# franciscospauldingastudillo/pyharp

Measured on AMD Instinct MI355X. Metric: DISORT column-solves/sec (nstr=16, nlyr=80); max |dF|/F vs cdisort, higher is better.
Workload: dtype f64

## Files before the change

pyharp_amd/csrc/hd_device.hpp:

```cpp
#pragma once

#include <hip/hip_runtime.h>

#ifndef HD_JACOBI_F32_ANGLE
#define HD_JACOBI_F32_ANGLE 1
#endif

namespace hd {

constexpr double kPi = 3.14159265358979323846;
constexpr double kDither = 4.712160915387242e-08;


constexpr double kResPolish = 3.0e-4;

constexpr double kResMove = 3.0e-8;
constexpr double kResClamp = 1.0e-9;
constexpr double kThinTau = 1.0e-3;

constexpr int kStBadInput = 0x01;
constexpr int kStEigen = 0x02;
constexpr int kStNonFinite = 0x04;
constexpr int kStResonance = 0x10;
constexpr int kStPivot = 0x20;

template <int NN>
struct Quad {
  double mu[NN];
  double w[NN];
  double sd[NN];
  double g[NN];
  double rmu[NN];
  double rg[NN];
  double pt[2 * NN][NN];
};

__device__ __forceinline__ double rcp_nr(double x) {
  double r = __builtin_amdgcn_rcp(x);
  double e = fma(-x, r, 1.0);
  r = fma(r, e, r);
  e = fma(-x, r, 1.0);
  return fma(r, e, r);
}

__device__ __forceinline__ double rsq_nr(double x) {
  double y = __builtin_amdgcn_rsq(x);
  const double h = 0.5 * x;
  double e = fma(-h * y, y, 0.5);
  y = fma(y, e, y);
  e = fma(-h * y, y, 0.5);
  return fma(y, e, y);
}

__device__ __forceinline__ double rsq_nr1(double x) {
  const double y = __builtin_amdgcn_rsq(x);
  const double e = fma(-0.5 * x * y, y, 0.5);
  return fma(y, e, y);
}

#define HD_SYM(a, i, j) a[((i) < (j) ? (i) : (j))][((i) < (j) ? (j) : (i))]

__device__ __forceinline__ double plkf(double x) { return x * x * x / expm1(x); }

__device__ inline double plkavg(double wlo, double whi, double t) {
  if (!(t >= 0.0) || !(whi > wlo) || wlo < 0.0) return __builtin_nan("");
  if (t < 1.0e-4) return 0.0;
  const double sigdpi = 5.67032e-8 / kPi;
  const double conc = 15.0 / (kPi * kPi * kPi * kPi);
  const double c2 = 1.438786;
  const double v0 = c2 * wlo / t, v1 = c2 * whi / t;
  const double t4 = t * t * t * t;
  if (v0 > 2.220446049250313e-16 && v1 < 709.782712893384 && (whi - wlo) / whi < 1.0e-2) {
    const double hh = v1 - v0;
    const double val0 = plkf(v0) + plkf(v1);
    double oldval = 0.0, val = 0.0;
    for (int n = 1; n <= 10; ++n) {
      const double del = hh / (2 * n);
      val = val0;
      for (int k = 1; k <= 2 * n - 1; ++k) val += 2 * (1 + k % 2) * plkf(v0 + k * del);
      val = del / 3.0 * val;
      if (fabs((val - oldval) / val) <= 1.0e-6) break;
      oldval = val;
    }
    return sigdpi * t4 * conc * val;
  }
  double pv[2] = {0.0, 0.0}, dv[2] = {0.0, 0.0};
  int smallv = 0;
#pragma unroll
  for (int i = 0; i < 2; ++i) {
    const double vi = i == 0 ? v0 : v1;
    if (vi < 1.5) {
      smallv++;
      const double vsq = vi * vi;
      pv[i] = conc * vsq * vi *
              (1.0 / 3.0 +
               vi * (-1.0 / 8.0 +
                     vi * (1.0 / 60.0 +
                           vsq * (-1.0 / 5040.0 +
                                  vsq * (1.0 / 272160.0 +
                                         vsq * (-1.0 / 13305600.0 + vsq * (1.0 / 622702080.0)))))));
    } else {
      const int mmax = vi >= 10.25 ? 1 : vi >= 5.7 ? 2 : vi >= 3.9 ? 3 : vi >= 2.9 ? 4
                       : vi >= 2.3 ? 5 : vi >= 1.9 ? 6 : 7;
      const double ex = exp(-vi);
      double exm = 1.0, di = 0.0;
      for (int m = 1; m <= mmax; ++m) {
        const double mv = m * vi;
        exm *= ex;
        const double m2 = (double)m * m;
        di += exm * (6.0 + mv * (6.0 + mv * (3.0 + mv))) / (m2 * m2);
      }
      dv[i] = conc * di;
    }
  }
  double val;
  if (smallv == 2) val = pv[1] - pv[0];
  else if (smallv == 1) val = 1.0 - pv[0] - dv[1];
  else val = dv[0] - dv[1];
  return sigdpi * t4 * val;
}


#ifndef HD_UNROLL_NN
#define HD_UNROLL_NN _Pragma("unroll")
#endif

template <int NN>
__device__ __forceinline__ bool chol_inplace(double (&a)[NN][NN], double (&rd)[NN]) {
  int ok = 1;
HD_UNROLL_NN
  for (int j = 0; j < NN; ++j) {
    double s = a[j][j];
HD_UNROLL_NN
    for (int k = 0; k < j; ++k) s = fma(-a[j][k], a[j][k], s);
    ok &= s > 0.0 ? 1 : 0;
    asm volatile("" : "+v"(ok));
    s = s > 1e-300 ? s : 1e-300;
    const double r = rsq_nr(s);
    a[j][j] = s * r;
    rd[j] = r;
HD_UNROLL_NN
    for (int i = j + 1; i < NN; ++i) {
      double t = a[j][i];
HD_UNROLL_NN
      for (int k = 0; k < j; ++k) t = fma(-a[i][k], a[j][k], t);
      a[i][j] = t * r;
    }
  }
  return ok != 0;
}

template <int NN>
__device__ __forceinline__ void lower_solve(const double (&l)[NN][NN], const double (&rd)[NN],
                                            double (&x)[NN]) {
HD_UNROLL_NN
  for (int i = 0; i < NN; ++i) {
    double s = x[i];
HD_UNROLL_NN
    for (int k = 0; k < i; ++k) s = fma(-l[i][k], x[k], s);
    x[i] = s * rd[i];
  }
}

template <int NN>
__device__ __forceinline__ void lower_t_solve(const double (&l)[NN][NN], const double (&rd)[NN],
                                              double (&x)[NN]) {
HD_UNROLL_NN
  for (int i = NN - 1; i >= 0; --i) {
    double s = x[i];
HD_UNROLL_NN
    for (int k = i + 1; k < NN; ++k) s = fma(-l[k][i], x[k], s);
    x[i] = s * rd[i];
  }
}

template <int NN>
__device__ __forceinline__ void spd_inverse_upper(double (&a)[NN][NN], const double (&rd)[NN]) {
  double k[NN][NN];
HD_UNROLL_NN
  for (int j = 0; j < NN; ++j) {
    k[j][j] = rd[j];
HD_UNROLL_NN
    for (int i = j + 1; i < NN; ++i) {
      double t = 0.0;
HD_UNROLL_NN
      for (int m = j; m < i; ++m) t = fma(a[i][m], k[m][j], t);
      k[i][j] = -t * rd[i];
    }
  }
HD_UNROLL_NN
  for (int i = 0; i < NN; ++i)
HD_UNROLL_NN
    for (int j = i; j < NN; ++j) {
      double t = 0.0;
HD_UNROLL_NN
      for (int m = j; m < NN; ++m) t = fma(k[m][i], k[m][j], t);
      a[i][j] = t;
    }
}

__host__ __device__ constexpr int tour_a(int P, int r, int k) {
  return k == 0 ? P - 1 : (r + k) % (P - 1);
}
__host__ __device__ constexpr int tour_b(int P, int r, int k) {
  return k == 0 ? r : (r - k + (P - 1)) % (P - 1);
}

template <int NN>
__device__ __forceinline__ void jacobi_round(int r, double (&a)[NN][NN], double (&v)[NN][NN],
                                             bool on) {
  constexpr int P = NN + (NN & 1);
  constexpr int H = P / 2;
  double cc[H], ss[H], tt[H];
HD_UNROLL_NN
  for (int k = 0; k < H; ++k) {
    const int x = tour_a(P, r, k), y = tour_b(P, r, k);
    const int p = x < y ? x : y, q = x < y ? y : x;
    if (q >= NN) continue;
    const double apq = a[p][q];
    const double d = a[q][q] - a[p][p];
    const double w2 = fma(d, d, 4.0 * apq * apq);
    const bool rot = on && w2 > 1.0e-280;
    const double w2s = rot ? w2 : 1.0;
    const double w = w2s * rsq_nr1(w2s);
    const double u = fabs(d) + w;
    const double z = rsq_nr1(2.0 * w * u);
    const double sg = d < 0.0 ? -2.0 : 2.0;
    cc[k] = rot ? u * z : 1.0;
    ss[k] = rot ? sg * apq * z : 0.0;
    tt[k] = rot ? sg * apq * (2.0 * w) * (z * z) : 0.0;
  }
HD_UNROLL_NN
  for (int k = 0; k < H; ++k) {
    const int x = tour_a(P, r, k), y = tour_b(P, r, k);
    const int p = x < y ? x : y, q = x < y ? y : x;
    if (q >= NN) continue;
    const double c = cc[k], s = ss[k], t = tt[k];
    const double apq = a[p][q];
    a[p][p] = fma(-t, apq, a[p][p]);
    a[q][q] = fma(t, apq, a[q][q]);
    a[p][q] = on ? 0.0 : apq;
HD_UNROLL_NN
    for (int i = 0; i < NN; ++i) {
      if (i == p || i == q) continue;
      const double aip = HD_SYM(a, i, p);
      const double aiq = HD_SYM(a, i, q);
      HD_SYM(a, i, p) = fma(c, aip, -s * aiq);
      HD_SYM(a, i, q) = fma(s, aip, c * aiq);
    }
HD_UNROLL_NN
    for (int i = 0; i < NN; ++i) {
      const double vip = v[i][p];
      const double viq = v[i][q];
      v[i][p] = fma(c, vip, -s * viq);
      v[i][q] = fma(s, vip, c * viq);
    }
  }
}

template <int NN>
__device__ __forceinline__ void jacobi_eig(double (&a)[NN][NN], double (&v)[NN][NN],
                                           int max_sweeps) {
HD_UNROLL_NN
  for (int i = 0; i < NN; ++i)
HD_UNROLL_NN
    for (int j = 0; j < NN; ++j) v[i][j] = (i == j) ? 1.0 : 0.0;
  if constexpr (NN > 1) {
    constexpr int P = NN + (NN & 1);
    for (int sweep = 0; sweep < max_sweeps; ++sweep) {
      double off = 0.0, dia = 0.0;
HD_UNROLL_NN
      for (int i = 0; i < NN; ++i) {
        dia = fma(a[i][i], a[i][i], dia);
HD_UNROLL_NN
        for (int j = i + 1; j < NN; ++j) off = fma(a[i][j], a[i][j], off);
      }
      const bool done = !(off > 1.0e-30 * dia);
      if (__all(done)) break;
HD_UNROLL_NN
      for (int r = 0; r < P - 1; ++r) jacobi_round<NN>(r, a, v, !done);
    }
  }
}

template <int NN, bool F64 = false>
__device__ __forceinline__ void jacobi_os_round(int r, double (&b)[NN][NN], double (&nrm)[NN],
                                                double (&sg)[NN], double (&rs)[NN], bool on,
                                                double& off) {
  constexpr int P = NN + (NN & 1);
  constexpr int H = P / 2;
  double tt[H], cc[H], gg[H];
HD_UNROLL_NN
  for (int k = 0; k < H; ++k) {
    const int x = tour_a(P, r, k), y = tour_b(P, r, k);
    const int p = x < y ? x : y, q = x < y ? y : x;
    if (q >= NN) continue;
    double g0 = 0.0, g1 = 0.0;
HD_UNROLL_NN
    for (int i = 0; i < NN; ++i) {
      if (i % 2 == 0) g0 = fma(b[i][p], b[i][q], g0);
      else g1 = fma(b[i][p], b[i][q], g1);
    }
    const double gam = (g0 + g1) * (sg[p] * sg[q]);
    const double app = nrm[p], aqq = nrm[q];
    off = fma(gam, gam, off);
    const double d = aqq - app;
    double t;
    if constexpr (HD_JACOBI_F32_ANGLE && !F64) {
      const float df = (float)d, g2f = 2.0f * (float)gam;
      const float wf = __builtin_amdgcn_sqrtf(__builtin_fmaf(g2f, g2f, df * df));
      const float dn = __builtin_fmaxf(__builtin_fabsf(df) + wf, 1.17549435e-38f);
      const float sn = __builtin_bit_cast(
          float, __builtin_bit_cast(unsigned, g2f) ^ (__builtin_bit_cast(unsigned, df) & 0x80000000u));
      const float nu = on ? sn : 0.0f;
      t = (double)(nu * __builtin_amdgcn_rcpf(dn));
    } else {
      const double g2 = gam * gam;
      const bool rot = on && g2 > 1.0e-30 * (app * aqq);
      const double w2 = rot ? fma(d, d, 4.0 * g2) : 1.0;
      const double w = w2 * rsq_nr(w2);
      t = rot ? (d < 0.0 ? -2.0 : 2.0) * gam * rcp_nr(fabs(d) + w) : 0.0;
    }
    tt[k] = t;
    cc[k] = F64 ? rsq_nr(fma(t, t, 1.0)) : rsq_nr1(fma(t, t, 1.0));
    gg[k] = gam;
  }
HD_UNROLL_NN
  for (int k = 0; k < H; ++k) {
    const int x = tour_a(P, r, k), y = tour_b(P, r, k);
    const int p = x < y ? x : y, q = x < y ? y : x;
    if (q >= NN) continue;
    const double t = tt[k], c = cc[k];
    const double al = -t * (sg[q] * rs[p]), be = t * (sg[p] * rs[q]);
HD_UNROLL_NN
    for (int i = 0; i < NN; ++i) {
      const double bp = b[i][p], bq = b[i][q];
      b[i][p] = fma(al, bq, bp);
      b[i][q] = fma(be, bp, bq);
    }
    const double rc = fma(t, t, 1.0) * c;
    sg[p] *= c;
    sg[q] *= c;
    rs[p] *= rc;
    rs[q] *= rc;
    nrm[p] = fma(-t, gg[k], nrm[p]);
    nrm[q] = fma(t, gg[k], nrm[q]);
  }
}

template <int NN>
__device__ __forceinline__ bool jacobi_os(double (&b)[NN][NN], int max_sweeps) {
  bool on = false;
  if constexpr (NN > 1) {
    constexpr int P = NN + (NN & 1);
    on = true;
    double sg[NN], rs[NN];
HD_UNROLL_NN
    for (int j = 0; j < NN; ++j) sg[j] = rs[j] = 1.0;
    for (int sweep = 0; sweep < max_sweeps; ++sweep) {
      double nrm[NN], dia = 0.0, off = 0.0;
HD_UNROLL_NN
      for (int j = 0; j < NN; ++j) {
        double t = 0.0;
HD_UNROLL_NN
        for (int i = 0; i < NN; ++i) t = fma(b[i][j], b[i][j], t);
        nrm[j] = t * (sg[j] * sg[j]);
        dia = fma(nrm[j], nrm[j], dia);
      }
HD_UNROLL_NN
      for (int r = 0; r < P - 1; ++r) jacobi_os_round<NN>(r, b, nrm, sg, rs, on, off);
      on = on && off > 1.0e-16 * dia;
      if (__all(!on)) break;
    }
HD_UNROLL_NN
    for (int j = 0; j < NN; ++j)
HD_UNROLL_NN
      for (int i = 0; i < NN; ++i) b[i][j] *= sg[j];
  }
  return !on;
}

template <int NN>
__device__ __forceinline__ bool jacobi_os_polish(double (&b)[NN][NN], bool need) {
  if constexpr (NN > 1) {
    if (!__any(need)) return false;
    constexpr int P = NN + (NN & 1);
    double sg[NN], rs[NN], nrm[NN], off = 0.0;
HD_UNROLL_NN
    for (int j = 0; j < NN; ++j) {
      sg[j] = rs[j] = 1.0;
      double t = 0.0;
HD_UNROLL_NN
      for (int i = 0; i < NN; ++i) t = fma(b[i][j], b[i][j], t);
      nrm[j] = t;
    }
HD_UNROLL_NN
    for (int r = 0; r < P - 1; ++r) jacobi_os_round<NN, true>(r, b, nrm, sg, rs, need, off);
HD_UNROLL_NN
    for (int j = 0; j < NN; ++j)
HD_UNROLL_NN
      for (int i = 0; i < NN; ++i) b[i][j] *= sg[j];
    return true;
  }
  return false;
}

template <int NN>
__device__ __forceinline__ void column_norms2(const double (&b)[NN][NN], double (&k2)[NN]) {
HD_UNROLL_NN
  for (int j = 0; j < NN; ++j) {
    double t = 0.0;
HD_UNROLL_NN
    for (int i = 0; i < NN; ++i) t = fma(b[i][j], b[i][j], t);
    k2[j] = t;
  }
}

template <int NN>
__device__ __forceinline__ bool near_resonance(const double (&k2)[NN], double r2, double tol) {
  bool near = false;
HD_UNROLL_NN
  for (int j = 0; j < NN; ++j) near = near || fabs(r2 - k2[j]) < tol * r2;
  return near;
}

}
```

pyharp_amd/csrc/hd_kernels.hip:

```cpp
#include <cmath>
#include <cstring>
#include <type_traits>
#include <utility>
#include <vector>

#include "hd_kernels.hpp"

namespace hd {

struct QuadTables {
  Quad<1> q1;
  Quad<2> q2;
  Quad<3> q3;
  Quad<4> q4;
  Quad<5> q5;
  Quad<6> q6;
  Quad<7> q7;
  Quad<8> q8;
};
__constant__ QuadTables c_quad;
__constant__ double c_quad_h[kMaxRegNN][kMaxRegNN];
template <int NN>
struct QuadS {
  double spt[2 * NN][NN];
// ... 199 lines not shown
      const double zj1 = z[j + 1];
      const double a1 = sqrt(fma(zj1 - zl, 2.0 * R + zj1 + zl, rm2));
      const double g = (2.0 * R + zj1 + zj) / (a1 + a0);
      if (j == l) g0 = g;
      sp = fma(dtp[(size_t)(L - 1 - j) * nsc + sl], g, sp);
      if (A.ch) su = fma(dtu[(size_t)(L - 1 - j) * nsc + sl], g, su);
      a0 = a1;
      zj = zj1;
    }
    A.chp[(size_t)lv * nsc + sl] = sp;
    if (A.ch) A.ch[(size_t)lv * nsc + sl] = su;
    const double dt = dtp[(size_t)(lv - 1) * nsc + sl];
    A.lam[(size_t)(lv - 1) * nsc + sl] = dt > 0.0 ? (sp - chp_top) / dt : g0;
    chp_top = sp;
  }
}

template <int NN>
__host__ __device__ constexpr int psi_doubles() {
  return NN > 1 ? (NN == 2 ? 5 : NN * NN) : 1;
}

template <int NN, bool NT, bool SPHER = false>
__device__ __forceinline__ int layer_body(const LayerArgs& A, long s, int sl, int lc,
                                          double* psi_lds, int lt, PairOutT<NT>& out,
                                          const double* pf = nullptr, float* pf_sink = nullptr,
                                          const SphArgs* P = nullptr) {
  constexpr int N = 2 * NN;
  constexpr int kPsi = psi_doubles<NN>();
  const Quad<NN>& Qc = quad<NN>();
  const int L = A.nlyr;
  const int nm = A.nmom;
  const int np = A.nprop;
  int st = 0;

  const double* q = A.prop + ((size_t)s * L + (L - 1 - lc)) * np;
  const double tau = q[0];
  double ssa = np > 1 ? q[1] : 0.0;
  if (!(tau >= 0.0) || !(ssa >= 0.0) || !(ssa <= 1.0)) st |= kStBadInput;
  if (ssa == 1.0) ssa = 1.0 - kDither;
  const double f = nm >= N ? q[1 + N] : 0.0;
  if (!(f < 1.0)) st |= kStBadInput;
  const double taup = (1.0 - ssa * f) * tau;
  const double om = ssa * (1.0 - f) / (1.0 - ssa * f);
  const double rf = om / (1.0 - f);

  const double mu0 = A.umu0 ? A.umu0[s] : 1.0;
  const double fb = A.fbeam ? A.fbeam[s] : 0.0;
  bool beam = fb > 0.0 && mu0 > 0.0;
  if (fb > 0.0 && !(mu0 > 0.0 && mu0 <= 1.0)) st |= kStBadInput;
  double rmu0 = beam ? 1.0 / mu0 : 0.0;
  if constexpr (SPHER) {
    beam = beam && P->chp[(size_t)(L + 1) * A.nsc + sl] != 0.0;
    rmu0 = beam ? P->lam[(size_t)lc * A.nsc + sl] : 0.0;
  }
  const double mub = beam ? mu0 : 0.0;

  const QuadS<NN>& Qs = quad_s<NN>();
  double lch[NN][NN], ap[NN][NN], xs[NN], xd[NN];
#pragma unroll
  for (int i = 0; i < NN; ++i) {
    xs[i] = xd[i] = 0.0;
#pragma unroll
    for (int j = i; j < NN; ++j) lch[i][j] = ap[i][j] = (i == j) ? Qc.rmu[i] : 0.0;
  }
  {
    double pprev = 0.0, pcur = 1.0;
#pragma nounroll
    for (int l2 = 0; l2 < NN; ++l2) {
      const int le = 2 * l2, lo = le + 1;
      const double che = le == 0 ? 1.0 : (le <= nm ? q[1 + le] : 0.0);
      const double cho = lo <= nm ? q[1 + lo] : 0.0;
      const double ge = -(2 * le + 1) * (che - f) * rf;
      const double go = -(2 * lo + 1) * (cho - f) * rf;
      const double pe0 = pcur;
      const double po0 = ((2 * lo - 1) * mub * pcur - (lo - 1) * pprev) * c_inv_int[lo];
      pprev = po0;
      pcur = ((2 * lo + 1) * mub * po0 - lo * pe0) * c_inv_int[lo + 1];
      double ue[NN], uo[NN];
#pragma unroll
      for (int i = 0; i < NN; ++i) {
        ue[i] = ge * Qs.spt[le][i];
        uo[i] = go * Qs.spt[lo][i];
        xs[i] = fma(ue[i], pe0, xs[i]);
        xd[i] = fma(uo[i], po0, xd[i]);
      }
#pragma unroll
      for (int i = 0; i < NN; ++i)
#pragma unroll
        for (int j = i; j < NN; ++j) {
          ap[i][j] = fma(ue[i], Qs.spt[le][j], ap[i][j]);
          lch[i][j] = fma(uo[i], Qs.spt[lo][j], lch[i][j]);
        }
    }
  }
  double rdl[NN];
  if (!chol_inplace<NN>(lch, rdl)) st |= kStEigen;

  double y2[NN], lxd[NN];
  const double fb2 = fb * (0.5 / kPi);
  if (beam) {
    double y[NN], z[NN];
#pragma unroll
    for (int i = 0; i < NN; ++i) y[i] = -fb2 * xs[i];
#pragma unroll
    for (int i = 0; i < NN; ++i) {
      double t = 0.0;
#pragma unroll
      for (int k = i; k < NN; ++k) t = fma(lch[k][i], y[k], t);
      z[i] = t;
    }
#pragma unroll
    for (int i = 0; i < NN; ++i) {
      double t = 0.0;
#pragma unroll
      for (int k = 0; k <= i; ++k) t = fma(lch[i][k], z[k], t);
      y[i] = t;
    }
#pragma unroll
    for (int i = 0; i < NN; ++i) {
      const double sxd = fb2 * xd[i];
      const double rv = fma(-y[i], Qc.rg[i], sxd * rmu0 * Qs.rmusd[i]);
      y2[i] = Qc.g[i] * rv;
      lxd[i] = sxd;
    }
    lower_solve<NN>(lch, rdl, y2);
    lower_solve<NN>(lch, rdl, lxd);
    lower_t_solve<NN>(lch, rdl, lxd);
  } else {
#pragma unroll
    for (int i = 0; i < NN; ++i) y2[i] = lxd[i] = 0.0;
  }
  double cvec[NN];
  double db = 0.0, bsum = 0.0;
  if (A.planck) {
    const double bt = A.planckv[(size_t)(L - lc) * A.nsc + sl];
    const double bb = taup > 0.0 ? A.planckv[(size_t)(L - lc - 1) * A.nsc + sl] : bt;
    db = bb - bt;
    bsum = bt + bb;
    const double b1 = taup > 0.0 ? 2.0 * db / taup : 0.0;
#pragma unroll
    for (int i = 0; i < NN; ++i) cvec[i] = Qc.sd[i] * Qc.mu[i];
    lower_solve<NN>(lch, rdl, cvec);
    lower_t_solve<NN>(lch, rdl, cvec);
#pragma unroll
    for (int i = 0; i < NN; ++i) cvec[i] = fma(b1 * Qc.rg[i], cvec[i], db);
  } else {
#pragma unroll
    for (int i = 0; i < NN; ++i) cvec[i] = 0.0;
  }

  double rdc[NN];
  if (!chol_inplace<NN>(ap, rdc)) st |= kStEigen;
  double v[NN][NN];
#pragma unroll
  for (int i = 0; i < NN; ++i)
#pragma unroll
    for (int j = 0; j < NN; ++j) {
      double t = 0.0;
#pragma unroll
      for (int k = (i > j ? i : j); k < NN; ++k) t = fma(lch[k][i], ap[k][j], t);
      v[i][j] = t;
    }
  constexpr int kPark = NN * (NN + 1) / 2 + NN;
  static_assert(kPark <= kPsi || NN == 1, "L does not fit the Psi staging area");
  if constexpr (NN > 1) {
    int e = 0;
#pragma unroll
    for (int i = 0; i < NN; ++i) {
#pragma unroll
      for (int k = 0; k <= i; ++k) psi_lds[(e++) * kLayerBlock + lt] = lch[i][k];
      psi_lds[(e++) * kLayerBlock + lt] = rdl[i];
    }
  }
  asm volatile("" ::: "memory");
#if HD_LAYER_PREFETCH
  if (pf) {
    using gp = const __attribute__((address_space(1))) void*;
    using lp = __attribute__((address_space(3))) void*;
    const int o1 = np > 16 ? 16 : np - 1, o2 = np > 17 ? 17 : np - 1;
    __builtin_amdgcn_global_load_lds((gp)(pf), (lp)(pf_sink), 4, 0, 0);
    __builtin_amdgcn_global_load_lds((gp)(pf + o1), (lp)(pf_sink), 4, 0, 0);
    __builtin_amdgcn_global_load_lds((gp)(pf + o2), (lp)(pf_sink), 4, 0, 0);
  }
#endif
  HD_PHASE();
  if (!jacobi_os<NN>(v, A.max_sweeps)) st |= kStEigen;
  double k2[NN];
  column_norms2<NN>(v, k2);
  if (jacobi_os_polish<NN>(v, beam && near_resonance<NN>(k2, rmu0 * rmu0, kResPolish)))
    column_norms2<NN>(v, k2);
  HD_PHASE();
  double kk[NN], rk[NN];
#pragma unroll
  for (int j = 0; j < NN; ++j) {
    if (!(k2[j] > 0.0)) st |= kStEigen;
    const double r = k2[j] > 0.0 ? rsq_nr(k2[j]) : 0.0;
    kk[j] = k2[j] * r;
    rk[j] = r;
  }
  double ybt[NN];
  double rmu0e = rmu0;
  if (beam) {
    double tt[NN];
    const double r2 = rmu0 * rmu0;
    bool near = false;
#pragma unroll
    for (int j = 0; j < NN; ++j) {
      double t = 0.0;
#pragma unroll
      for (int i = 0; i < NN; ++i) t = fma(v[i][j], y2[i], t);
      double den = fma(-kk[j], kk[j], r2);
      if constexpr (SPHER) {
        if (fabs(den) < kResClamp * r2) {
          st |= kStResonance;
          den = den < 0.0 ? -kResClamp * r2 : kResClamp * r2;
        }
      } else {
        near = near || fabs(den) < kResMove * r2;
      }
      tt[j] = t * (rk[j] * rk[j]) * rcp_nr(den);
    }
    if constexpr (!SPHER) {
      if (near) {
        st |= kStResonance;
        double dmin = 2.0 * r2, r2e = r2;
#pragma unroll
        for (int j = 0; j < NN; ++j) {
          const double den = fma(-kk[j], kk[j], r2);
          if (fabs(den) < dmin) {
            dmin = fabs(den);
            r2e = kk[j] * kk[j] * (den < 0.0 ? 1.0 - kResMove : 1.0 + kResMove);
          }
        }
        rmu0e = sqrt(r2e);
#pragma unroll
        for (int j = 0; j < NN; ++j) {
          double t = 0.0;
#pragma unroll
          for (int i = 0; i < NN; ++i) t = fma(v[i][j], y2[i], t);
          tt[j] = t * (rk[j] * rk[j]) * rcp_nr(fma(-kk[j], kk[j], r2e));
        }
      }
    }
#pragma unroll
    for (int i = 0; i < NN; ++i) {
      double t = 0.0;
#pragma unroll
      for (int j = 0; j < NN; ++j) t = fma(v[i][j], tt[j], t);
      ybt[i] = t;
    }
  }
  HD_PHASE();
  if constexpr (NN > 1) {
    asm volatile("" ::: "memory");
    int e = 0;
#pragma unroll
    for (int i = 0; i < NN; ++i) {
#pragma unroll
      for (int k = 0; k <= i; ++k) lch[i][k] = psi_lds[(e++) * kLayerBlock + lt];
      rdl[i] = psi_lds[(e++) * kLayerBlock + lt];
    }
  }
  HD_PHASE();

  double zp[NN], zm[NN];
  double e0 = 0.0;
  if (beam) {
    double sv[NN], y[NN];
#pragma unroll
    for (int i = NN - 1; i >= 0; --i) {
      double t = 0.0;
#pragma unroll
      for (int k = 0; k <= i; ++k) t = fma(lch[i][k], ybt[k], t);
      sv[i] = Qc.rg[i] * t;
    }
#pragma unroll
    for (int i = 0; i < NN; ++i) y[i] = Qc.sd[i] * Qc.mu[i] * sv[i];
    lower_solve<NN>(lch, rdl, y);
    lower_t_solve<NN>(lch, rdl, y);
    double att;
    if constexpr (SPHER) {
      const double ct = P->chp[(size_t)lc * A.nsc + sl];
      att = 0.5 * exp(-ct);
      e0 = taup > 0.0 ? exp(ct - P->chp[(size_t)(lc + 1) * A.nsc + sl]) : 1.0;
    } else {
      const double tauc = A.tauc ? A.tauc[(size_t)lc * A.nsc + sl] : 0.0;
      att = 0.5 * exp(-tauc * rmu0);
    }
#pragma unroll
    for (int i = 0; i < NN; ++i) {
      const double dd = Qc.rg[i] * fma(-y[i], rmu0e, lxd[i]);
      zp[i] = (sv[i] + dd) * att;
      zm[i] = (sv[i] - dd) * att;
    }
    if constexpr (!SPHER) e0 = exp(-taup * rmu0e);
  } else {
#pragma unroll
    for (int i = 0; i < NN; ++i) zp[i] = zm[i] = 0.0;
  }

  HD_PHASE();
  double dsq[NN];
#pragma unroll
  for (int j = 0; j < NN; ++j) {
    const double x = kk[j] * taup;
    const double m = -expm1(-x);
    const double th = m * rcp_nr(2.0 - m);
    const double delta = x > 1.0e-8 ? th * rcp_nr(kk[j] > 0.0 ? kk[j] : 1.0) : 0.5 * taup;
    dsq[j] = delta > 0.0 ? delta * rsq_nr1(delta) : 0.0;
  }
#pragma unroll
  for (int j = 0; j < NN; ++j) {
    double x[NN];
#pragma unroll
    for (int i = 0; i < NN; ++i) x[i] = v[i][j] * dsq[j];
    lower_t_solve<NN>(lch, rdl, x);
#pragma unroll
    for (int i = 0; i < NN; ++i) psi_lds[(i * NN + j) * kLayerBlock + lt] = x[i];
  }
  HD_PHASE();
#pragma unroll
  for (int j = 0; j < NN; ++j) {
    const double sc = rk[j] * dsq[j];
#pragma unroll
    for (int i = 0; i < NN; ++i) v[i][j] *= sc;
  }
#pragma unroll
  for (int i = NN - 1; i >= 0; --i)
#pragma unroll
    for (int j = 0; j < NN; ++j) {
      double t = 0.0;
#pragma unroll
      for (int k = 0; k <= i; ++k) t = fma(lch[i][k], v[k][j], t);
      v[i][j] = t;
    }
  HD_PHASE();

  using RL = RecL<NN>;
  constexpr int nsym = NN * (NN + 1) / 2;
  double ga[NN], gb[NN];
#pragma unroll
  for (int i = 0; i < NN; ++i) {
    ga[i] = Qc.g[i] * (cvec[i] - fma(-zp[i], e0, zm[i]));
    gb[i] = Qc.g[i] * (fma(zp[i], e0, zm[i]) + bsum);
  }
  const bool thin = A.planck && taup > 0.0 && taup < kThinTau;
  if (thin) {
    double y[NN];
#pragma unroll
    for (int j = 0; j < NN; ++j) {
      double t = 0.0;
#pragma unroll
      for (int i = 0; i < NN; ++i) t = fma(v[i][j], Qc.g[i] * (cvec[i] - db), t);
      y[j] = t;
    }
#pragma unroll
    for (int i = 0; i < NN; ++i) {
      double t = 0.0;
#pragma unroll
      for (int j = 0; j < NN; ++j) t = fma(v[i][j], y[j], t);
      ga[i] = Qc.g[i] * (db - fma(-zp[i], e0, zm[i])) - t;
    }
  }
  double pvec[NN], am_[NN][NN];
  {
#pragma unroll
    for (int i = 0; i < NN; ++i)
#pragma unroll
      for (int j = i; j < NN; ++j) {
        double t = (i == j) ? 1.0 : 0.0;
#pragma unroll
        for (int k = 0; k < NN; ++k) t = fma(v[i][k], v[j][k], t);
        am_[i][j] = t;
      }
    double rdh[NN];
    if (!chol_inplace<NN>(am_, rdh)) st |= kStEigen;
    spd_inverse_upper<NN>(am_, rdh);
#pragma unroll
    for (int i = 0; i < NN; ++i) {
      double t = ga[i];
#pragma unroll
      for (int j = 0; j < NN; ++j) t = fma(-HD_SYM(am_, i, j), ga[j], t);
      pvec[i] = t;
    }
    if (thin) {
#pragma unroll
      for (int i = 0; i < NN; ++i) pvec[i] += Qc.g[i] * (db - fma(-zp[i], e0, zm[i])) - ga[i];
    }
  }
  double ap_[NN][NN], qvec[NN];
  {
    double pt_[NN][NN];
#pragma unroll
    for (int i = 0; i < NN; ++i)
#pragma unroll
      for (int j = 0; j < NN; ++j) pt_[i][j] = psi_lds[(i * NN + j) * kLayerBlock + lt];
#pragma unroll
    for (int i = 0; i < NN; ++i)
#pragma unroll
      for (int j = i; j < NN; ++j) {
        double t = (i == j) ? 1.0 : 0.0;
#pragma unroll
        for (int k = 0; k < NN; ++k) t = fma(pt_[i][k], pt_[j][k], t);
        ap_[i][j] = t;
      }
    double rdh[NN];
    if (!chol_inplace<NN>(ap_, rdh)) st |= kStEigen;
    spd_inverse_upper<NN>(ap_, rdh);
#pragma unroll
    for (int i = 0; i < NN; ++i) {
      double t = -gb[i];
#pragma unroll
      for (int j = 0; j < NN; ++j) t = fma(HD_SYM(ap_, i, j), gb[j], t);
      qvec[i] = t;
    }
  }

  double chk = 0.0;
  {
    int e = 0;
#pragma unroll
    for (int i = 0; i < NN; ++i)
#pragma unroll
      for (int j = i; j < NN; ++j, ++e) {
        const double r = ap_[i][j] - am_[i][j];
        out.put(RL::R + e, r);
        chk += r;
      }
    out.close(RL::R + nsym - 1);
    e = 0;
#pragma unroll
    for (int i = 0; i < NN; ++i)
#pragma unroll
      for (int j = i; j < NN; ++j, ++e) {
        const double t = (am_[i][j] + ap_[i][j]) - ((i == j) ? 1.0 : 0.0);
        out.put(RL::T + e, t);
        chk += t;
      }
    out.close(RL::T + nsym - 1);
  }
  double smv[NN];
#pragma unroll
  for (int i = 0; i < NN; ++i) {
    const double sp = Qc.g[i] * (zp[i] * (1.0 - e0) - db) + pvec[i] - qvec[i];
    smv[i] = Qc.g[i] * (-zm[i] * (1.0 - e0) + db) - pvec[i] - qvec[i];
    out.put(RL::Sp + i, sp);
    chk += sp + smv[i];
  }
  out.close(RL::Sp + NN - 1);
#pragma unroll
  for (int i = 0; i < NN; ++i) out.put(RL::Sm + i, smv[i]);
  out.close(RL::Sm + NN - 1);
  out.put(RL::Tau, taup);
  out.close(RL::Tau);
  if (!isfinite(chk + taup)) st |= kStNonFinite;
  return st;
}

template <int NN, bool NT>
__global__ __launch_bounds__(kLayerBlock) void hd_layer_kernel(LayerArgs A) {
  __shared__ double psi_lds[psi_doubles<NN>() * kLayerBlock];
  const int lt = threadIdx.x;
  const int ntl = (A.nlyr + kLayersPerBlock - 1) / kLayersPerBlock;
  const int nb = (int)gridDim.x;
  auto tile_of = [&](int b, int& ts, int& tl) {
    const int x = b & 7, base = nb >> 3, extra = nb & 7;
    const int logical = x * base + (x < extra ? x : extra) + (b >> 3);
    ts = logical / ntl;
    tl = logical - ts * ntl;
  };
  int ts, tl;
  tile_of((int)blockIdx.x, ts, tl);
  const int sl = ts * 64 + (lt & 63);
  const int lc = tl * kLayersPerBlock + (lt >> 6);
  if (sl >= A.nsc || lc >= A.nlyr) return;
  const long s = solve_of(A.s0 + sl, A.cmaj, A.nwave, A.ncol);
  PairOutT<NT> out{reinterpret_cast<double2*>(A.scr) + (size_t)lc * RecL<NN>::pairs * A.nsc + sl,
                   (size_t)A.nsc, 0.0};
#if HD_LAYER_PREFETCH
  __shared__ float pf_sink[kLayerBlock];
  const double* pf = nullptr;
  if ((int)blockIdx.x + HD_LAYER_PREFETCH < nb) {
    int ts2, tl2;
    tile_of((int)blockIdx.x + HD_LAYER_PREFETCH, ts2, tl2);
    int sl2 = ts2 * 64 + (lt & 63);
    const int lc2 = tl2 * kLayersPerBlock + (lt >> 6);
    if (sl2 >= A.nsc) sl2 = A.nsc - 1;
    if (lc2 < A.nlyr) {
      const long s2 = solve_of(A.s0 + sl2, A.cmaj, A.nwave, A.ncol);
      pf = A.prop + ((size_t)s2 * A.nlyr + (A.nlyr - 1 - lc2)) * A.nprop;
    }
  }
  const int st =
      layer_body<NN, NT>(A, s, sl, lc, psi_lds, lt, out, pf, pf_sink);
#else
  const int st =
      layer_body<NN, NT>(A, s, sl, lc, psi_lds, lt, out);
#endif
  if (st) {
    atomicOr(&A.status[s], st);
    if (st & 0x0F) atomicOr(A.anyerr, 1);
  }
}
template <int NN, bool NT>
__global__ __launch_bounds__(kLayerBlock) void hd_layer_spher_kernel(LayerArgs A, SphArgs P) {
  __shared__ double psi_lds[psi_doubles<NN>() * kLayerBlock];
  const int lt = threadIdx.x;
  const int ntl = (A.nlyr + kLayersPerBlock - 1) / kLayersPerBlock;
  const int nb = (int)gridDim.x;
  auto tile_of = [&](int b, int& ts, int& tl) {
    const int x = b & 7, base = nb >> 3, extra = nb & 7;
    const int logical = x * base + (x < extra ? x : extra) + (b >> 3);
    ts = logical / ntl;
    tl = logical - ts * ntl;
  };
  int ts, tl;
  tile_of((int)blockIdx.x, ts, tl);
  const int sl = ts * 64 + (lt & 63);
  const int lc = tl * kLayersPerBlock + (lt >> 6);
  if (sl >= A.nsc || lc >= A.nlyr) return;
  const long s = solve_of(A.s0 + sl, A.cmaj, A.nwave, A.ncol);
  PairOutT<NT> out{reinterpret_cast<double2*>(A.scr) + (size_t)lc * RecL<NN>::pairs * A.nsc + sl,
                   (size_t)A.nsc, 0.0};
#if HD_LAYER_PREFETCH
  __shared__ float pf_sink[kLayerBlock];
  const double* pf = nullptr;
  if ((int)blockIdx.x + HD_LAYER_PREFETCH < nb) {
    int ts2, tl2;
    tile_of((int)blockIdx.x + HD_LAYER_PREFETCH, ts2, tl2);
    int sl2 = ts2 * 64 + (lt & 63);
    const int lc2 = tl2 * kLayersPerBlock + (lt >> 6);
    if (sl2 >= A.nsc) sl2 = A.nsc - 1;
    if (lc2 < A.nlyr) {
      const long s2 = solve_of(A.s0 + sl2, A.cmaj, A.nwave, A.ncol);
      pf = A.prop + ((size_t)s2 * A.nlyr + (A.nlyr - 1 - lc2)) * A.nprop;
    }
  }
  const int st =
      layer_body<NN, NT, true>(A, s, sl, lc, psi_lds, lt, out, pf, pf_sink, &P);
#else
  const int st =
      layer_body<NN, NT, true>(A, s, sl, lc, psi_lds, lt, out, nullptr, nullptr, &P);
#endif
  if (st) {
    atomicOr(&A.status[s], st);
    if (st & 0x0F) atomicOr(A.anyerr, 1);
  }
}
__device__ __forceinline__ void flx_emit(const FlxArgs& F, long s, long sl, size_t nsc, int L,
                                         int lc, double up, double dn, double uavgup,
                                         double uavgdn, double blev) {
  const size_t nl = (size_t)(L + 1) * nsc;
  const double rfldir = F.lvl[(size_t)lc * nsc + sl];
  const double uavgso = F.lvl[nl + (size_t)lc * nsc + sl];
  const double absl = F.lvl[2 * nl + (size_t)lc * nsc + sl];
  const double uavg = uavgup + uavgdn + uavgso;
  double* o = F.flx + ((size_t)s * (L + 1) + (L - lc)) * kNFlx;
  double2* o2 = reinterpret_cast<double2*>(o);
  o2[0] = make_double2(rfldir, dn - rfldir);
  o2[1] = make_double2(up, absl * (uavg - blev));
  o2[2] = make_double2(uavg, uavgdn);
  o2[3] = make_double2(uavgup, uavgso);
}

template <int NN, bool NT, bool FLX = false, bool SPHER = false, class RecAt>
__device__ __forceinline__ int sweep_body(const SweepArgs& A, long sl, long s, RecAt&& rec_at,
                                          const FlxArgs* F = nullptr, const SphArgs* P = nullptr) {
  const Quad<NN>& Qc = quad<NN>();
  const int L = A.nlyr;
  const size_t nsc = A.nsc;
  constexpr int nsym = NN * (NN + 1) / 2;
  int st = 0;

  const double mu0 = A.umu0 ? A.umu0[s] : 1.0;
  const double fb = A.fbeam ? A.fbeam[s] : 0.0;
  bool beam = fb > 0.0 && mu0 > 0.0;
  if constexpr (SPHER) beam = beam && P->chp[(size_t)(L + 1) * nsc + sl] != 0.0;
  const double alb = A.albedo ? A.albedo[s] : 0.0;
  if (!(alb >= 0.0) || !(alb <= 1.0)) st |= kStBadInput;
  double top = A.fisot ? A.fisot[s] : 0.0;
  double bsurf = 0.0;
  if (A.planck) {
    bsurf = A.planckv[(size_t)(L + 1) * nsc + sl];
    top += A.planckv[(size_t)(L + 2) * nsc + sl];
  }
  const double twopi = 2.0 * kPi;
  const double rmu0 = beam ? 1.0 / mu0 : 0.0;
  const double f0mu0 = beam ? fb * mu0 : 0.0;
  auto beam_at = [&](int lc, double tauc) {
    if constexpr (SPHER) return beam ? exp(-P->chp[(size_t)lc * nsc + sl]) : 1.0;
    else return exp(-tauc * rmu0);
  };

  double ra[NN][NN];
  double sd[NN];
#pragma unroll
  for (int i = 0; i < NN; ++i) {
    sd[i] = Qc.g[i] * top;
#pragma unroll
    for (int j = i; j < NN; ++j) ra[i][j] = 0.0;
  }
  double tauc = 0.0;

  for (int lc = 0; lc < L; ++lc) {
    using RL = RecL<NN>;
    using RB = std::conditional_t<FLX, RecBF<NN>, RecB<NN>>;
    auto rec = rec_at(lc);
    PairOutT<NT> bp{reinterpret_cast<double2*>(A.bsub) + (size_t)lc * RB::pairs * nsc + sl, nsc, 0.0};
    double rl[NN][NN], spl[NN];
    {
      int e = 0;
#pragma unroll
      for (int i = 0; i < NN; ++i)
#pragma unroll
        for (int j = i; j < NN; ++j) rl[i][j] = rec(RL::R + (e++));
#pragma unroll
      for (int i = 0; i < NN; ++i) spl[i] = rec(RL::Sp + i);
    }
    const double eb = beam_at(lc, tauc);
    const double sscale = A.beam_scale ? eb : 1.0;
#pragma unroll
    for (int i = 0; i < NN; ++i) spl[i] *= sscale;

    {
      double cs = 0.0;
#pragma unroll
      for (int i = 0; i < NN; ++i) {
        double t = 0.0;
#pragma unroll
        for (int j = 0; j < NN; ++j) t = fma(HD_SYM(ra, j, i), Qc.g[j], t);
        bp.put(RB::Rc + i, twopi * t);
        cs = fma(Qc.g[i], sd[i], cs);
      }
      bp.close(RB::Rc + NN - 1);
      bp.put(RB::Cs, fma(twopi, cs, f0mu0 * eb));
      bp.close(RB::Cs);
    }
    if constexpr (FLX) {
      double ch = 0.0;
#pragma unroll
      for (int i = 0; i < NN; ++i) {
        double t = 0.0;
#pragma unroll
        for (int j = 0; j < NN; ++j) t = fma(HD_SYM(ra, j, i), c_quad_h[NN - 1][j], t);
        bp.put(RB::Rh + i, t);
        ch = fma(c_quad_h[NN - 1][i], sd[i], ch);
      }
      bp.close(RB::Rh + NN - 1);
      bp.put(RB::Ch, ch);
      bp.close(RB::Ch);
    }
    HD_PHASE();
    double am[NN][NN], w1[NN][NN], t1[NN];
#pragma unroll
    for (int i = 0; i < NN; ++i)
#pragma unroll
      for (int j = 0; j < NN; ++j) am[i][j] = HD_SYM(ra, i, j);
#pragma unroll
    for (int i = 0; i < NN; ++i) {
#pragma unroll
      for (int j = 0; j < NN; ++j) {
        double t = (i == j) ? 1.0 : 0.0;
#pragma unroll
        for (int k = 0; k < NN; ++k) t = fma(-HD_SYM(rl, i, k), am[k][j], t);
        w1[i][j] = t;
      }
      double t = spl[i];
#pragma unroll
      for (int k = 0; k < NN; ++k) t = fma(HD_SYM(rl, i, k), sd[k], t);
      t1[i] = t;
    }
    HD_PHASE();
#pragma unroll
    for (int k = 0; k < NN; ++k) {
      const double piv = w1[k][k];
      if (!(fabs(piv) > 1.0e-12)) st |= kStPivot;
      const double rp = rcp_nr(piv);
      w1[k][k] = rp;
#pragma unroll
      for (int i = k + 1; i < NN; ++i) {
        const double l = w1[i][k] * rp;
        w1[i][k] = l;
#pragma unroll
        for (int j = k + 1; j < NN; ++j) w1[i][j] = fma(-l, w1[k][j], w1[i][j]);
      }
    }
#pragma unroll
    for (int i = 0; i < NN; ++i)
#pragma unroll
      for (int k = 0; k < i; ++k) t1[i] = fma(-w1[i][k], t1[k], t1[i]);
#pragma unroll
    for (int i = NN - 1; i >= 0; --i) {
#pragma unroll
      for (int k = i + 1; k < NN; ++k) t1[i] = fma(-w1[i][k], t1[k], t1[i]);
      t1[i] *= w1[i][i];
    }
    double u[NN];
#pragma unroll
    for (int i = 0; i < NN; ++i) {
      double t = sd[i];
#pragma unroll
      for (int k = 0; k < NN; ++k) t = fma(am[i][k], t1[k], t);
      u[i] = t;
      bp.put(RB::Tv + i, t1[i]);
    }
    bp.close(RB::Tv + NN - 1);
    HD_PHASE();
#pragma unroll
    for (int r = 0; r < NN; ++r) {
#pragma unroll
      for (int j = 0; j < NN; ++j) {
        double t = am[r][j];
#pragma unroll
        for (int k = 0; k < j; ++k) t = fma(-am[r][k], w1[k][j], t);
        am[r][j] = t * w1[j][j];
      }
#pragma unroll
      for (int j = NN - 1; j >= 0; --j) {
        double t = am[r][j];
#pragma unroll
        for (int k = j + 1; k < NN; ++k) t = fma(-am[r][k], w1[k][j], t);
        am[r][j] = t;
      }
    }
    HD_PHASE();
    double tl[NN][NN];
    {
      int e = 0;
#pragma unroll
      for (int i = 0; i < NN; ++i)
#pragma unroll
        for (int j = i; j < NN; ++j) tl[i][j] = rec(RL::T + (e++));
    }
    {
      double sm_[NN];
#pragma unroll
      for (int i = 0; i < NN; ++i) sm_[i] = rec(RL::Sm + i);
      const double taul = rec(RL::Tau);
#pragma unroll
      for (int i = 0; i < NN; ++i) {
        double t = sm_[i] * sscale;
#pragma unroll
        for (int k = 0; k < NN; ++k) t = fma(HD_SYM(tl, i, k), u[k], t);
        sd[i] = t;
      }
      tauc += taul;
    }
#pragma unroll
    for (int j = 0; j < NN; ++j) {
      double x[NN];
#pragma unroll
      for (int i = 0; i < NN; ++i) x[i] = HD_SYM(tl, i, j);
#pragma unroll
      for (int i = 0; i < NN; ++i)
#pragma unroll
        for (int k = 0; k < i; ++k) x[i] = fma(-w1[i][k], x[k], x[i]);
#pragma unroll
      for (int i = NN - 1; i >= 0; --i) {
#pragma unroll
        for (int k = i + 1; k < NN; ++k) x[i] = fma(-w1[i][k], x[k], x[i]);
        x[i] *= w1[i][i];
      }
#pragma unroll
      for (int i = 0; i < NN; ++i) bp.put(RB::Z + j * NN + i, x[i]);
    }
    bp.close(RB::Z + NN * NN - 1);
    HD_PHASE();
#pragma unroll
    for (int r = 0; r < NN; ++r) {
      double row[NN];
#pragma unroll
      for (int j = 0; j < NN; ++j) {
        double t = 0.0;
#pragma unroll
        for (int k = 0; k < NN; ++k) t = fma(am[r][k], HD_SYM(tl, k, j), t);
        row[j] = t;
      }
#pragma unroll
      for (int j = 0; j < NN; ++j) am[r][j] = row[j];
    }
    HD_PHASE();
#pragma unroll
    for (int i = 0; i < NN; ++i) {
#pragma unroll
      for (int j = i; j < NN; ++j) {
        double t = rl[i][j];
#pragma unroll
        for (int k = 0; k < NN; ++k) t = fma(HD_SYM(tl, i, k), am[k][j], t);
        ra[i][j] = t;
      }
    }
  }

  double gsd = 0.0, grg = 0.0;
#pragma unroll
  for (int i = 0; i < NN; ++i) {
    gsd += Qc.g[i] * sd[i];
#pragma unroll
    for (int j = 0; j < NN; ++j) grg += Qc.g[i] * HD_SYM(ra, i, j) * Qc.g[j];
  }
  double esurf = (1.0 - alb) * bsurf;
  const double dirsurf = f0mu0 * beam_at(L, tauc);
  if (beam) esurf += alb * dirsurf / kPi;
  const double x = (2.0 * alb * gsd + esurf) / (1.0 - 2.0 * alb * grg);
  double ip[NN];
#pragma unroll
  for (int i = 0; i < NN; ++i) ip[i] = Qc.g[i] * x;
  double chk = 0.0;
  {
    double up = 0.0, dn = 0.0;
#pragma unroll
    for (int i = 0; i < NN; ++i) {
      up += Qc.g[i] * ip[i];
      double t = sd[i];
#pragma unroll
      for (int j = 0; j < NN; ++j) t += HD_SYM(ra, i, j) * ip[j];
      dn += Qc.g[i] * t;
    }
    const double f0 = twopi * up, f1 = twopi * dn + dirsurf;
    if (A.flux) {
      double* fo = A.flux + (size_t)s * (L + 1) * 2;
      fo[0] = f0;
      fo[1] = f1;
    }
    if (A.fsurf) {
      A.fsurf[sl] = f0;
      A.fsurf[nsc + sl] = f1;
    }
    chk += f0 + f1;
    if constexpr (FLX) {
      double hu = 0.0, hd_ = 0.0;
#pragma unroll
      for (int i = 0; i < NN; ++i) {
        const double h = c_quad_h[NN - 1][i];
        hu = fma(h, ip[i], hu);
        double t = sd[i];
#pragma unroll
        for (int j = 0; j < NN; ++j) t += HD_SYM(ra, i, j) * ip[j];
        hd_ = fma(h, t, hd_);
      }
      const double bl = A.planck ? A.planckv[sl] : 0.0;
      flx_emit(*F, s, sl, nsc, L, L, f0, f1, 0.5 * hu, 0.5 * hd_, bl);
    }
  }
  A.xsurf[sl] = x;
  if (!isfinite(chk)) st |= kStNonFinite;
  return st;
}

template <int NN, bool NT>
__global__ __launch_bounds__(64) void hd_sweep_kernel(SweepArgs A) {
  const long sl = (long)blockIdx.x * blockDim.x + threadIdx.x;
  if (sl >= A.nsc) return;
  const long s = solve_of(A.s0 + sl, A.cmaj, A.nwave, A.ncol);
  const size_t nsc = A.nsc;
  auto rec_at = [&](int lc) {
    const double2* lp =
        reinterpret_cast<const double2*>(A.scr) + (size_t)lc * RecL<NN>::pairs * nsc + sl;
    return [lp, nsc](int e) { return pair_get<NT>(lp, nsc, e); };
  };
  const int st = sweep_body<NN, NT>(A, sl, s, rec_at);
  if (st) {
    atomicOr(&A.status[s], st);
    if (st & 0x0F) atomicOr(A.anyerr, 1);
  }
}

template <int NN, bool NT, bool FLX>
__global__ __launch_bounds__(64) void hd_sweep_spher_kernel(SweepArgs A, FlxArgs F, SphArgs P) {
  const long sl = (long)blockIdx.x * blockDim.x + threadIdx.x;
  if (sl >= A.nsc) return;
  const long s = solve_of(A.s0 + sl, A.cmaj, A.nwave, A.ncol);
  const size_t nsc = A.nsc;
  auto rec_at = [&](int lc) {
    const double2* lp =
        reinterpret_cast<const double2*>(A.scr) + (size_t)lc * RecL<NN>::pairs * nsc + sl;
    return [lp, nsc](int e) { return pair_get<NT>(lp, nsc, e); };
  };
  const int st = sweep_body<NN, NT, FLX, true>(A, sl, s, rec_at, &F, &P);
  if (st) {
    atomicOr(&A.status[s], st);
    if (st & 0x0F) atomicOr(A.anyerr, 1);
  }
}

template <int NN, bool NT>
__global__ __launch_bounds__(64) void hd_sweep_flx_kernel(SweepArgs A, FlxArgs F) {
  const long sl = (long)blockIdx.x * blockDim.x + threadIdx.x;
  if (sl >= A.nsc) return;
  const long s = A.s0 + sl;
  const size_t nsc = A.nsc;
  auto rec_at = [&](int lc) {
    const double2* lp =
        reinterpret_cast<const double2*>(A.scr) + (size_t)lc * RecL<NN>::pairs * nsc + sl;
    return [lp, nsc](int e) { return pair_get<NT>(lp, nsc, e); };
  };
  const int st = sweep_body<NN, NT, true>(A, sl, s, rec_at, &F);
  if (st) {
    atomicOr(&A.status[s], st);
    if (st & 0x0F) atomicOr(A.anyerr, 1);
  }
}

template <int NN, bool PRE, bool NT, bool FLX = false>
__device__ __forceinline__ void backsub_body(const SweepArgs& A, const FlxArgs* F = nullptr);


namespace {
template <int NN, int K>
__device__ __forceinline__ double qbc(double x) {
  constexpr int ctrl = NN == 4 ? (K | (K << 2) | (K << 4) | (K << 6))
                               : (K | (K << 2) | ((2 + K) << 4) | ((2 + K) << 6));
  return __builtin_amdgcn_update_dpp(0.0, x, ctrl, 0xF, 0xF, true);
}
template <int NN>
__device__ __forceinline__ double qsum(double x) {
  x += __builtin_amdgcn_update_dpp(0.0, x, 1 | (0 << 2) | (3 << 4) | (2 << 6), 0xF, 0xF, true);
  if constexpr (NN == 4)
    x += __builtin_amdgcn_update_dpp(0.0, x, 2 | (3 << 2) | (0 << 4) | (1 << 6), 0xF, 0xF, true);
  return x;
}
template <int B, int E, class F, int... Is>
__device__ __forceinline__ void qfor_impl(F&& f, std::integer_sequence<int, Is...>) {
  (f(std::integral_constant<int, B + Is>{}), ...);
}
template <int B, int E, class F>
__device__ __forceinline__ void qfor(F&& f) {
  if constexpr (E > B) qfor_impl<B, E>(f, std::make_integer_sequence<int, E - B>{});
}
#define HD_Q(x) decltype(x)::value
}

template <int NN>
__global__ __launch_bounds__(64) void hd_sweep_quad_kernel(SweepArgs A) {
  static_assert(NN == 2 || NN == 4, "pair / quad teams");
  const Quad<NN>& Qc = quad<NN>();
  const int lane = (int)threadIdx.x;
  const int i = lane & (NN - 1);
  const long slq = ((long)blockIdx.x * 64 + lane) / NN;
  const bool valid = slq < A.nsc;
  const long sl = valid ? slq : A.nsc - 1;
  const long s = solve_of(A.s0 + sl, A.cmaj, A.nwave, A.ncol);
  const int L = A.nlyr;
  const size_t nsc = A.nsc;
  using RL = RecL<NN>;
  using RB = RecB<NN>;
  int st = 0;

  const double mu0 = A.umu0 ? A.umu0[s] : 1.0;
  const double fb = A.fbeam ? A.fbeam[s] : 0.0;
  const bool beam = fb > 0.0 && mu0 > 0.0;
  const double alb = A.albedo ? A.albedo[s] : 0.0;
  if (!(alb >= 0.0) || !(alb <= 1.0)) st |= kStBadInput;
  double top = A.fisot ? A.fisot[s] : 0.0;
  double bsurf = 0.0;
  if (A.planck) {
    bsurf = A.planckv[(size_t)(L + 1) * nsc + sl];
    top += A.planckv[(size_t)(L + 2) * nsc + sl];
  }
  const double twopi = 2.0 * kPi;
  const double rmu0 = beam ? 1.0 / mu0 : 0.0;
  const double f0mu0 = beam ? fb * mu0 : 0.0;
  const double g_i = Qc.g[i];
  auto eoff = [&](int e) { return ((size_t)(e >> 1) * nsc + sl) * 2 + (e & 1); };

  double ra[NN];
#pragma unroll
  for (int j = 0; j < NN; ++j) ra[j] = 0.0;
  double sd = g_i * top;
  double tauc = 0.0;

  double rn[NN], tn[NN], spn, smn, tpn;
  auto fetch = [&](int lc) {
    const double* lb = A.scr + (size_t)lc * RL::pairs * nsc * 2;
#pragma unroll
    for (int j = 0; j < NN; ++j) {
      rn[j] = lb[eoff(RL::R + sym_index<NN>(i, j))];
      tn[j] = lb[eoff(RL::T + sym_index<NN>(i, j))];
    }
    spn = lb[eoff(RL::Sp + i)];
    smn = lb[eoff(RL::Sm + i)];
    tpn = lb[eoff(RL::Tau)];
  };
  fetch(0);
  for (int lc = 0; lc < L; ++lc) {
    double* bb = A.bsub + (size_t)lc * RB::pairs * nsc * 2;
    double r[NN], tr[NN];
#pragma unroll
    for (int j = 0; j < NN; ++j) {
      r[j] = rn[j];
      tr[j] = tn[j];
    }
    const double eb = exp(-tauc * rmu0);
    const double sscale = A.beam_scale ? eb : 1.0;
    const double spl = spn * sscale;
    const double sml = smn * sscale;
    const double taup = tpn;
    fetch(lc + 1 < L ? lc + 1 : lc);

    {
      double rc = 0.0;
#pragma unroll
      for (int j = 0; j < NN; ++j) rc = fma(ra[j], Qc.g[j], rc);
      const double cs = qsum<NN>(g_i * sd);
      if (valid) {
        bb[eoff(RB::Rc + i)] = twopi * rc;
        if (i == 0) bb[eoff(RB::Cs)] = fma(twopi, cs, f0mu0 * eb);
      }
    }
    double w[NN];
#pragma unroll
    for (int j = 0; j < NN; ++j) w[j] = i == j ? 1.0 : 0.0;
    double v = spl;
    qfor<0, NN>([&](auto K) {
      constexpr int k = HD_Q(K);
#pragma unroll
      for (int j = 0; j < NN; ++j) w[j] = fma(-r[k], qbc<NN, k>(ra[j]), w[j]);
      v = fma(r[k], qbc<NN, k>(sd), v);
    });
    double z[NN], d = 1.0;
#pragma unroll
    for (int j = 0; j < NN; ++j) z[j] = tr[j];
    qfor<0, NN>([&](auto K) {
      constexpr int k = HD_Q(K);
      const double pk = qbc<NN, k>(w[k]);
      st |= fabs(pk) > 1.0e-12 ? 0 : kStPivot;
      d = i == k ? pk : d;
      const double f = i == k ? 0.0 : w[k] * rcp_nr(pk);
      qfor<k + 1, NN>([&](auto J) { w[HD_Q(J)] = fma(-f, qbc<NN, k>(w[HD_Q(J)]), w[HD_Q(J)]); });
#pragma unroll
      for (int j = 0; j < NN; ++j) z[j] = fma(-f, qbc<NN, k>(z[j]), z[j]);
      v = fma(-f, qbc<NN, k>(v), v);
    });
    {
      const double rd = rcp_nr(d);
#pragma unroll
      for (int j = 0; j < NN; ++j) z[j] *= rd;
      v *= rd;
    }
    if (valid) {
#pragma unroll
      for (int j = 0; j < NN; ++j) bb[eoff(RB::Z + j * NN + i)] = z[j];
      bb[eoff(RB::Tv + i)] = v;
    }
    double u = sd, p_[NN];
#pragma unroll
    for (int j = 0; j < NN; ++j) p_[j] = 0.0;
    qfor<0, NN>([&](auto K) {
      constexpr int k = HD_Q(K);
      u = fma(ra[k], qbc<NN, k>(v), u);
#pragma unroll
      for (int j = 0; j < NN; ++j) p_[j] = fma(ra[k], qbc<NN, k>(z[j]), p_[j]);
    });
    double sdn = sml;
#pragma unroll
    for (int j = 0; j < NN; ++j) ra[j] = r[j];
    qfor<0, NN>([&](auto K) {
      constexpr int k = HD_Q(K);
#pragma unroll
      for (int j = 0; j < NN; ++j) ra[j] = fma(tr[k], qbc<NN, k>(p_[j]), ra[j]);
      sdn = fma(tr[k], qbc<NN, k>(u), sdn);
    });
    sd = sdn;
    tauc += taup;
  }

  double rgi = 0.0;
#pragma unroll
  for (int j = 0; j < NN; ++j) rgi = fma(ra[j], Qc.g[j], rgi);
  const double gsd = qsum<NN>(g_i * sd);
  const double grg = qsum<NN>(g_i * rgi);
  double esurf = (1.0 - alb) * bsurf;
  const double dirsurf = f0mu0 * exp(-tauc * rmu0);
  if (beam) esurf += alb * dirsurf / kPi;
  const double x = (2.0 * alb * gsd + esurf) / (1.0 - 2.0 * alb * grg);
  const double up = qsum<NN>(g_i * (g_i * x));
  const double dn = qsum<NN>(g_i * fma(rgi, x, sd));
  const double f0 = twopi * up, f1 = twopi * dn + dirsurf;
  if (valid && i == 0) {
    if (A.flux) {
      double* fo = A.flux + (size_t)s * (L + 1) * 2;
      fo[0] = f0;
      fo[1] = f1;
    }
    if (A.fsurf) {
      A.fsurf[sl] = f0;
      A.fsurf[nsc + sl] = f1;
    }
    A.xsurf[sl] = x;
  }
  if (!isfinite(f0 + f1)) st |= kStNonFinite;
  if (valid && st && i == 0) {
// ... 500 lines not shown
```

Before: 15.21 million.

## Vectorize expm1 in eigen scaling and cut register pressure in doubling recursion

Replaces the per-element library expm1 with a custom batched polynomial exp(-x) evaluation across all NN eigenvalues, and reuses precomputed reciprocal eigenvalues rk instead of recomputing them. In the adding/doubling step it drops the full am copy of ra, computes only the upper triangle of the symmetric product m1 via row-wise triangular solves, and for NN>4 fuses the two matrix products column by column so no full NN×NN intermediate is live. The aim is fewer live registers (less spilling) and cheaper transcendental math, at the cost of a hand-rolled expm1 whose accuracy differs slightly from the library and relies on m1 being symmetric.

```diff
diff --git a/pyharp_amd/csrc/hd_device.hpp b/pyharp_amd/csrc/hd_device.hpp
--- a/pyharp_amd/csrc/hd_device.hpp
+++ b/pyharp_amd/csrc/hd_device.hpp
@@ -1,6 +1,54 @@
 #pragma once
 
+#ifdef HD_DEVICE_HOST_MATH
+#include <cmath>
+#define HD_HOST_DEVICE inline
+#define HD_UNROLL
+#else
 #include <hip/hip_runtime.h>
+#define HD_HOST_DEVICE __host__ __device__ __forceinline__
+#define HD_UNROLL _Pragma("unroll")
+#endif
+
+namespace hd {
+
+template <int N>
+HD_HOST_DEVICE void hd_m_expm1_neg_n(const double (&x)[N], double (&m)[N]) {
+  double r[N], s[N], q[N];
+HD_UNROLL
+  for (int j = 0; j < N; ++j) {
+    const double xc = fmin(x[j], 708.0);
+    const double fn = rint(xc * 1.4426950408889634);
+    r[j] = fma(-fn, 2.3190468138462996e-17, fma(-fn, 0.6931471805599453, xc));
+    const long long bits = (long long)(1023 - (int)fn) << 52;
+    __builtin_memcpy(&s[j], &bits, sizeof(double));
+    q[j] = -1.6059043836821613e-10;
+  }
+  constexpr double c[11] = {2.08767569878681e-09,  -2.505210838544172e-08, 2.755731922398589e-07,
+                            -2.7557319223985893e-06, 2.48015873015873e-05, -0.0001984126984126984,
+                            0.001388888888888889,  -0.008333333333333333,  0.041666666666666664,
+                            -0.16666666666666666,  0.5};
+HD_UNROLL
+  for (int k = 0; k < 11; ++k)
+HD_UNROLL
+    for (int j = 0; j < N; ++j) q[j] = fma(q[j], r[j], c[k]);
+HD_UNROLL
+  for (int j = 0; j < N; ++j) {
+    const double p = fma(r[j] * r[j], q[j], -r[j]);
+    m[j] = fma(-s[j], p, 1.0 - s[j]);
+  }
+}
+
+HD_HOST_DEVICE double hd_m_expm1_neg(double x) {
+  const double xs[1] = {x};
+  double ms[1];
+  hd_m_expm1_neg_n<1>(xs, ms);
+  return ms[0];
+}
+
+}
+
+#ifndef HD_DEVICE_HOST_MATH
 
 #ifndef HD_JACOBI_F32_ANGLE
 #define HD_JACOBI_F32_ANGLE 1
@@ -425,3 +473,5 @@
 }
 
 }
+
+#endif
diff --git a/pyharp_amd/csrc/hd_kernels.hip b/pyharp_amd/csrc/hd_kernels.hip
--- a/pyharp_amd/csrc/hd_kernels.hip
+++ b/pyharp_amd/csrc/hd_kernels.hip
@@ -525,12 +525,18 @@
 
   HD_PHASE();
   double dsq[NN];
+  double kt[NN], em[NN];
+#pragma unroll
+  for (int j = 0; j < NN; ++j) kt[j] = kk[j] * taup;
+  hd_m_expm1_neg_n<NN>(kt, em);
+#pragma unroll
+  for (int j = 0; j < NN; ++j) asm volatile("" : "+v"(em[j]));
 #pragma unroll
   for (int j = 0; j < NN; ++j) {
-    const double x = kk[j] * taup;
-    const double m = -expm1(-x);
+    const double x = kt[j];
+    const double m = em[j];
     const double th = m * rcp_nr(2.0 - m);
-    const double delta = x > 1.0e-8 ? th * rcp_nr(kk[j] > 0.0 ? kk[j] : 1.0) : 0.5 * taup;
+    const double delta = x > 1.0e-8 ? th * rk[j] : 0.5 * taup;
     dsq[j] = delta > 0.0 ? delta * rsq_nr1(delta) : 0.0;
   }
 #pragma unroll
@@ -875,18 +881,14 @@
       bp.close(RB::Ch);
     }
     HD_PHASE();
-    double am[NN][NN], w1[NN][NN], t1[NN];
-#pragma unroll
-    for (int i = 0; i < NN; ++i)
-#pragma unroll
-      for (int j = 0; j < NN; ++j) am[i][j] = HD_SYM(ra, i, j);
+    double w1[NN][NN], t1[NN];
 #pragma unroll
     for (int i = 0; i < NN; ++i) {
 #pragma unroll
       for (int j = 0; j < NN; ++j) {
         double t = (i == j) ? 1.0 : 0.0;
 #pragma unroll
-        for (int k = 0; k < NN; ++k) t = fma(-HD_SYM(rl, i, k), am[k][j], t);
+        for (int k = 0; k < NN; ++k) t = fma(-HD_SYM(rl, i, k), HD_SYM(ra, k, j), t);
         w1[i][j] = t;
       }
       double t = spl[i];
@@ -924,27 +926,30 @@
     for (int i = 0; i < NN; ++i) {
       double t = sd[i];
 #pragma unroll
-      for (int k = 0; k < NN; ++k) t = fma(am[i][k], t1[k], t);
+      for (int k = 0; k < NN; ++k) t = fma(HD_SYM(ra, i, k), t1[k], t);
       u[i] = t;
       bp.put(RB::Tv + i, t1[i]);
     }
     bp.close(RB::Tv + NN - 1);
     HD_PHASE();
+    double m1[NN][NN];
 #pragma unroll
     for (int r = 0; r < NN; ++r) {
+      double z[NN];
 #pragma unroll
       for (int j = 0; j < NN; ++j) {
-        double t = am[r][j];
-#pragma unroll
-        for (int k = 0; k < j; ++k) t = fma(-am[r][k], w1[k][j], t);
-        am[r][j] = t * w1[j][j];
-      }
-#pragma unroll
-      for (int j = NN - 1; j >= 0; --j) {
-        double t = am[r][j];
-#pragma unroll
-        for (int k = j + 1; k < NN; ++k) t = fma(-am[r][k], w1[k][j], t);
-        am[r][j] = t;
+        double t = HD_SYM(ra, r, j);
+#pragma unroll
+        for (int k = 0; k < j; ++k) t = fma(-z[k], w1[k][j], t);
+        z[j] = t * w1[j][j];
+      }
+#pragma unroll
+      for (int j = NN - 1; j >= r; --j) {
+        double t = z[j];
+#pragma unroll
+        for (int k = j + 1; k < NN; ++k) t = fma(-z[k], w1[k][j], t);
+        z[j] = t;
+        m1[r][j] = t;
       }
     }
     HD_PHASE();
@@ -990,28 +995,47 @@
     }
     bp.close(RB::Z + NN * NN - 1);
     HD_PHASE();
-#pragma unroll
-    for (int r = 0; r < NN; ++r) {
-      double row[NN];
+    if constexpr (NN > 4) {
 #pragma unroll
       for (int j = 0; j < NN; ++j) {
-        double t = 0.0;
-#pragma unroll
-        for (int k = 0; k < NN; ++k) t = fma(am[r][k], HD_SYM(tl, k, j), t);
-        row[j] = t;
-      }
-#pragma unroll
-      for (int j = 0; j < NN; ++j) am[r][j] = row[j];
-    }
-    HD_PHASE();
-#pragma unroll
-    for (int i = 0; i < NN; ++i) {
-#pragma unroll
-      for (int j = i; j < NN; ++j) {
-        double t = rl[i][j];
-#pragma unroll
-        for (int k = 0; k < NN; ++k) t = fma(HD_SYM(tl, i, k), am[k][j], t);
-        ra[i][j] = t;
+        double pc[NN];
+#pragma unroll
+        for (int r = 0; r < NN; ++r) {
+          double t = 0.0;
+#pragma unroll
+          for (int k = 0; k < NN; ++k) t = fma(HD_SYM(m1, r, k), HD_SYM(tl, k, j), t);
+          pc[r] = t;
+        }
+#pragma unroll
+        for (int i = 0; i <= j; ++i) {
+          double t = rl[i][j];
+#pragma unroll
+          for (int k = 0; k < NN; ++k) t = fma(HD_SYM(tl, i, k), pc[k], t);
+          ra[i][j] = t;
+        }
+      }
+    } else {
+      double pm[NN][NN];
+#pragma unroll
+      for (int r = 0; r < NN; ++r) {
+#pragma unroll
+        for (int j = 0; j < NN; ++j) {
+          double t = 0.0;
+#pragma unroll
+          for (int k = 0; k < NN; ++k) t = fma(HD_SYM(m1, r, k), HD_SYM(tl, k, j), t);
+          pm[r][j] = t;
+        }
+      }
+      HD_PHASE();
+#pragma unroll
+      for (int i = 0; i < NN; ++i) {
+#pragma unroll
+        for (int j = i; j < NN; ++j) {
+          double t = rl[i][j];
+#pragma unroll
+          for (int k = 0; k < NN; ++k) t = fma(HD_SYM(tl, i, k), pm[k][j], t);
+          ra[i][j] = t;
+        }
       }
     }
   }
```

Result: faster. 15.50 million (median of 6 runs) (+1.9%).
